# kerry-he/fsae-mpc

Hardware: AMD Instinct MI355X
Metric: QP solves/sec (batched LTV-MPC, N=40 nx=5 nu=2 fp64) (higher is better)
Workload: dtype f64

## Files before the change

### fsae-mpc_amd/csrc/qp_solver.hip

```cpp
#include <hip/hip_runtime.h>
#include <math.h>
#include <stdint.h>
#include <stdlib.h>
#include <stdio.h>
#include "qp_solver.h"

typedef double v4d __attribute__((ext_vector_type(4)));
typedef double v2d __attribute__((ext_vector_type(2)));

#define DEVINL __device__ __forceinline__
#ifndef QP_SOLVE_REFINE_STEPS
#define QP_SOLVE_REFINE_STEPS 1
#endif
#ifndef QP_FULL_BARRIERS
#define WAVE_SYNC() do { __builtin_amdgcn_fence(__ATOMIC_SEQ_CST, "wavefront"); __builtin_amdgcn_wave_barrier(); } while (0)
#else
#define WAVE_SYNC() __syncthreads()
#endif

namespace {

DEVINL double rl(double v, int src) {
  int lo = __builtin_amdgcn_readlane(__double2loint(v), src);
  int hi = __builtin_amdgcn_readlane(__double2hiint(v), src);
// ... 403 lines not shown
}

template <int T> DEVINL void hx_from_acc(const Ctx& k, const v4d* acc, const double* XV, double* HX) {
  double xr[T][4], xc[T], sc[T], sr[T][4];
#pragma unroll
  for (int I = 0; I < T; ++I) {
    xc[I] = XV[16 * I + k.c]; sc[I] = 0.0;
#pragma unroll
    for (int p = 0; p < 4; ++p) { xr[I][p] = XV[16 * I + k.q + 4 * p]; sr[I][p] = 0.0; }
  }
#pragma unroll
  for (int I = 0; I < T; ++I)
#pragma unroll
    for (int J = I; J < T; ++J) {
      const v4d& h = acc[Tri<T>::idx(I, J)];
#pragma unroll
      for (int p = 0; p < 4; ++p) {
        sc[J] = fma(h[p], xr[I][p], sc[J]);
        if (J > I) sr[I][p] = fma(h[p], xc[J], sr[I][p]);
      }
    }
  WAVE_SYNC();
#pragma unroll
  for (int J = 0; J < T; ++J) { const double v = q_sum(sc[J]); if (k.q == 0) HX[16 * J + k.c] = v; }
  WAVE_SYNC();
#pragma unroll
  for (int I = 0; I < T - 1; ++I)
#pragma unroll
    for (int p = 0; p < 4; ++p) { const double v = grp16_sum(sr[I][p]); if (k.c == 0) HX[16 * I + k.q + 4 * p] += v; }
}

template <int C> struct IC { static constexpr int value = C; };

#ifdef QP_DRAIN_STREAM
template <int T> struct StreamCfg {
  static constexpr int R = 3 * T;
};
template <int T> struct Stream {
  static constexpr int R = StreamCfg<T>::R;
  const char* gnext;
  int half;
  DEVINL void issue(const Ctx& k, int slot) {
    __builtin_amdgcn_global_load_lds((const __attribute__((address_space(1))) void*)(gnext + k.lane * 16),
                                     (__attribute__((address_space(3))) void*)(k.ring + slot * 128), 16, 0, 0);
    gnext += 1024;
  }
  DEVINL void start(const Ctx& k, int c0) {
    gnext = reinterpret_cast<const char*>(k.Aw); half = 0;
#pragma unroll
    for (int t = 0; t < T; ++t) if (t < c0) issue(k, t);
  }
  template <int C> DEVINL void next_pair(const Ctx& k, v2d* b, int cn) {
    asm volatile("s_waitcnt vmcnt(0)" ::: "memory");
    const int other = (half ^ 1) * T;
#pragma unroll
    for (int t = 0; t < T; ++t) if (t < cn) issue(k, other + t);
    asm volatile("" ::: "memory");
#pragma unroll
    for (int t = 0; t < C; ++t) b[t] = *reinterpret_cast<const v2d*>(k.ring + (half * T + t) * 128 + k.lane * 2);
    half ^= 1;
  }
  DEVINL void drain() { asm volatile("s_waitcnt vmcnt(0)" ::: "memory"); }
};
#else
template <int T> struct StreamCfg {
  static constexpr int D = 2 * T;
  static constexpr int R = D + T;
};
template <int T> struct Stream {
  static constexpr int D = StreamCfg<T>::D, R = StreamCfg<T>::R;
  const char* gnext; int slot_i, slot_e;
  DEVINL void issue(const Ctx& k) {
    __builtin_amdgcn_global_load_lds((const __attribute__((address_space(1))) void*)(gnext + k.lane * 16),
                                     (__attribute__((address_space(3))) void*)(k.ring + slot_i * 128), 16, 0, 0);
    gnext += 1024;
    slot_i = slot_i + 1 == R ? 0 : slot_i + 1;
  }
  DEVINL void start(const Ctx& k, int) {
    gnext = reinterpret_cast<const char*>(k.Aw); slot_i = 0; slot_e = 0;
#pragma unroll
    for (int j = 0; j < D; ++j) issue(k);
  }
  template <int C> DEVINL void next_pair(const Ctx& k, v2d* b, int) {
#pragma unroll
    for (int t = 0; t < C; ++t) issue(k);
    asm volatile("s_waitcnt vmcnt(%0)" :: "n"(D) : "memory");
#pragma unroll
    for (int t = 0; t < C; ++t) {
      int sl = slot_e + t; if (sl >= R) sl -= R;
      b[t] = *reinterpret_cast<const v2d*>(k.ring + sl * 128 + k.lane * 2);
    }
    slot_e += C; if (slot_e >= R) slot_e -= R;
  }
  DEVINL void drain() { asm volatile("s_waitcnt vmcnt(0)" ::: "memory"); }
};
#endif

template <int NA> struct CoefStage {
  double reg[NA > 0 ? NA : 1];
  DEVINL void load(const Ctx& k, const double* const* arr, int js) {
    const int jc = js < k.J ? js : k.J - 1;
#pragma unroll
    for (int a = 0; a < NA; ++a) reg[a] = arr[a][jc * 64 + k.lane];
  }
  DEVINL void commit(const Ctx& k) {
#pragma unroll
    for (int a = 0; a < NA; ++a) k.cof[a * 64 + k.lane] = reg[a];
  }
  DEVINL void read_pair(const Ctx& k, int s, v2d* out) const {
#pragma unroll
    for (int a = 0; a < NA; ++a) out[a] = *reinterpret_cast<const v2d*>(k.cof + a * 64 + k.q * 16 + (s & 15));
  }
};

template <int T, int NB> DEVINL void pass_syrk(const Ctx& k, v4d* acc, double* P1, double* P2, double* P3, double* MB) {
  constexpr int NBB = NB > 0 ? NB : 1;
  constexpr int NA = 4 + NB;
  const int JS = k.J * 64;
  const double* arr[NA];
  arr[0] = rowp(k, R_D); arr[1] = rowp(k, R_W1); arr[2] = rowp(k, R_W2); arr[3] = rowp(k, R_W3);
#pragma unroll
  for (int e = 0; e < NB; ++e) arr[4 + e] = k.Ab + (size_t)e * JS;
  double p1[T], p2[T], p3[T];
  double pb[NBB][T], sbb[NBB][NBB], pwb[3][NBB];
#pragma unroll
  for (int t = 0; t < T; ++t) { p1[t] = 0; p2[t] = 0; p3[t] = 0; }
#pragma unroll
  for (int e = 0; e < NBB; ++e) {
#pragma unroll
    for (int t = 0; t < T; ++t) pb[e][t] = 0;
#pragma unroll
    for (int f = 0; f < NBB; ++f) sbb[e][f] = 0;
    pwb[0][e] = pwb[1][e] = pwb[2][e] = 0;
  }
  Stream<T> st;
  CoefStage<NA> cs;
  int tr = 0;
  if (k.ntr > 0) { st.start(k, k.tcs[0]); cs.load(k, arr, 0); }
  auto phase = [&](auto Cc) __attribute__((always_inline)) {
    constexpr int C = decltype(Cc)::value;
    const int tr_end = k.tend[C];
    for (; tr < tr_end; ++tr) {
      if ((tr & 3) == 0) { cs.commit(k); cs.load(k, arr, (tr >> 2) + 1); }
#pragma unroll
      for (int u = 0; u < 2; ++u) {
        v2d b[C], cf[NA];
        st.template next_pair<C>(k, b, u == 0 ? C : (tr + 1 < tr_end ? C : (tr + 1 < k.ntr ? k.tcs[tr + 1] : 0)));
        cs.read_pair(k, 4 * tr + 2 * u, cf);
        asm volatile("" ::: "memory");
#pragma unroll
        for (int h = 0; h < 2; ++h) {
          double a[C], ab[NBB];
          const double dd = cf[0][h], w1 = cf[1][h], w2 = cf[2][h], w3 = cf[3][h];
#pragma unroll
          for (int e = 0; e < NB; ++e) ab[e] = cf[4 + e][h];
#pragma unroll
          for (int t = 0; t < C; ++t) a[t] = dd * b[t][h];
#pragma unroll
          for (int I = 0; I < C; ++I)
#pragma unroll
            for (int Jt = I; Jt < C; ++Jt)
              acc[Tri<T>::idx(I, Jt)] = __builtin_amdgcn_mfma_f64_16x16x4f64(a[I], b[Jt][h], acc[Tri<T>::idx(I, Jt)], 0, 0, 0);
#pragma unroll
          for (int t = 0; t < C; ++t) {
            p1[t] = fma(w1, b[t][h], p1[t]); p2[t] = fma(w2, b[t][h], p2[t]); p3[t] = fma(w3, b[t][h], p3[t]);
          }
#pragma unroll
          for (int e = 0; e < NB; ++e) {
            const double dab = dd * ab[e];
#pragma unroll
            for (int t = 0; t < C; ++t) pb[e][t] = fma(dab, b[t][h], pb[e][t]);
#pragma unroll
            for (int f = e; f < NB; ++f) sbb[e][f] = fma(dab, ab[f], sbb[e][f]);
            pwb[0][e] = fma(w1, ab[e], pwb[0][e]); pwb[1][e] = fma(w2, ab[e], pwb[1][e]); pwb[2][e] = fma(w3, ab[e], pwb[2][e]);
          }
        }
      }
    }
  };
  if constexpr (T >= 1) phase(IC<1>{});
  if constexpr (T >= 2) phase(IC<2>{});
  if constexpr (T >= 3) phase(IC<3>{});
  if constexpr (T >= 4) phase(IC<4>{});
  if constexpr (T >= 5) phase(IC<5>{});
  if constexpr (T >= 6) phase(IC<6>{});
  if constexpr (T >= 7) phase(IC<7>{});
  if constexpr (T >= 8) phase(IC<8>{});
  if (k.ntr > 0) st.drain();
#pragma unroll
  for (int t = 0; t < T; ++t) {
    double v1 = q_sum(p1[t]), v2 = q_sum(p2[t]), v3 = q_sum(p3[t]);
    if (k.q == 0) { P1[16 * t + k.c] = v1; P2[16 * t + k.c] = v2; P3[16 * t + k.c] = v3; }
  }
#pragma unroll
  for (int e = 0; e < NB; ++e) {
#pragma unroll
    for (int t = 0; t < T; ++t) { const double vb = q_sum(pb[e][t]); if (k.q == 0) MB[e * k.np + 16 * t + k.c] = vb; }
    const double v1 = q_sum(pwb[0][e]), v2 = q_sum(pwb[1][e]), v3 = q_sum(pwb[2][e]);
    if (k.lane == 0) { P1[k.nc + e] = v1; P2[k.nc + e] = v2; P3[k.nc + e] = v3; }
#pragma unroll
    for (int f = 0; f < NB; ++f) {
      const double sv = q_sum(f >= e ? sbb[e][f] : sbb[f][e]);
      if (k.lane == 0) MB[e * k.np + k.nc + f] = sv;
    }
  }
}

template <int T, int NB, int NVEC, int FUSE> DEVINL void pass_Av(const Ctx& k, const double* const* vin, double* const* rout, double* Pcor, double* Pcor2 = nullptr, const double* const* cfarr = nullptr) {
  constexpr int NBB = NB > 0 ? NB : 1;
  constexpr int NC = FUSE == 1 ? 6 : (FUSE >= 2 ? 3 : 0);
  constexpr int NA = NC + NB;
  const int JS = k.J * 64;
  const double* arr[NA > 0 ? NA : 1];
  if (FUSE == 1) { arr[0] = rowp(k, R_RPL); arr[1] = rowp(k, R_CB1); arr[2] = rowp(k, R_CC1); arr[3] = rowp(k, R_RPU); arr[4] = rowp(k, R_CB2); arr[5] = rowp(k, R_CC2); }
  if (FUSE >= 2) { arr[0] = cfarr ? cfarr[0] : rowp(k, R_CB1); arr[1] = cfarr ? cfarr[1] : rowp(k, R_RPL); arr[2] = cfarr ? cfarr[2] : rowp(k, R_CC1); }
#pragma unroll
  for (int f = 0; f < NB; ++f) arr[NC + f] = k.Ab + (size_t)f * JS;
  double v[NVEC][T], vb[NVEC][NBB], pc[T], pcb[NBB], pd[FUSE >= 2 ? T : 1], pdb[NBB];
#pragma unroll
  for (int e = 0; e < NVEC; ++e) {
#pragma unroll
    for (int t = 0; t < T; ++t) v[e][t] = vin[e][16 * t + k.c];
#pragma unroll
    for (int f = 0; f < NB; ++f) vb[e][f] = vin[e][k.nc + f];
  }
#pragma unroll
  for (int t = 0; t < T; ++t) pc[t] = 0.0;
#pragma unroll
  for (int f = 0; f < NBB; ++f) { pcb[f] = 0.0; pdb[f] = 0.0; }
#pragma unroll
  for (int t = 0; t < (FUSE >= 2 ? T : 1); ++t) pd[t] = 0.0;
  double keep[NVEC + 1];
#pragma unroll
  for (int e = 0; e < NVEC + 1; ++e) keep[e] = 0.0;
  Stream<T> st;
  CoefStage<NA> cs;
  int tr = 0;
  if (k.ntr > 0) { st.start(k, k.tcs[0]); if (NA > 0) cs.load(k, arr, 0); }
  auto phase = [&](auto Cc) __attribute__((always_inline)) {
    constexpr int C = decltype(Cc)::value;
    const int tr_end = k.tend[C];
    for (; tr < tr_end; ++tr) {
      if (NA > 0 && (tr & 3) == 0) { cs.commit(k); cs.load(k, arr, (tr >> 2) + 1); }
#pragma unroll
      for (int u = 0; u < 2; ++u) {
        v2d b[C], cf[NA > 0 ? NA : 1];
        st.template next_pair<C>(k, b, u == 0 ? C : (tr + 1 < tr_end ? C : (tr + 1 < k.ntr ? k.tcs[tr + 1] : 0)));
        if (NA > 0) cs.read_pair(k, 4 * tr + 2 * u, cf);
        asm volatile("" ::: "memory");
#pragma unroll
        for (int h = 0; h < 2; ++h) {
          const int s = 4 * tr + 2 * u + h;
          const int cc = s & 15;
#pragma unroll
          for (int e = 0; e < NVEC; ++e) {
            double dsum = 0.0;
#pragma unroll
            for (int t = 0; t < C; ++t) dsum = fma(b[t][h], v[e][t], dsum);
            dsum = grp16_sum(dsum);
#pragma unroll
            for (int f = 0; f < NB; ++f) dsum = fma(cf[NC + f][h], vb[e][f], dsum);
            if (k.c == cc) keep[e] = dsum;
            if (FUSE >= 2 && e == 0) {
              const double pen = cf[0][h] * (dsum - cf[1][h]);
              const double ynew = cf[2][h] - pen;
              if (k.c == cc) keep[NVEC] = ynew;
#pragma unroll
              for (int t = 0; t < C; ++t) { pc[t] = fma(ynew, b[t][h], pc[t]); pd[t] = fma(pen, b[t][h], pd[t]); }
#pragma unroll
              for (int f = 0; f < NB; ++f) { pcb[f] = fma(ynew, cf[NC + f][h], pcb[f]); pdb[f] = fma(pen, cf[NC + f][h], pdb[f]); }
            }
            if (FUSE == 1 && e == 0) {
              const double dl_ = dsum + cf[0][h], du_ = cf[3][h] - dsum;
              const double w = dl_ * fma(cf[2][h], dl_, cf[1][h]) - du_ * fma(cf[5][h], du_, cf[4][h]);
#pragma unroll
              for (int t = 0; t < C; ++t) pc[t] = fma(w, b[t][h], pc[t]);
#pragma unroll
              for (int f = 0; f < NB; ++f) pcb[f] = fma(w, cf[NC + f][h], pcb[f]);
            }
          }
          if (cc == 15 || s + 1 == 4 * k.ntr) {
            const int js = s >> 4;
#pragma unroll
            for (int e = 0; e < NVEC; ++e) { rout[e][js * 64 + k.lane] = keep[e]; keep[e] = 0.0; }
            if (FUSE >= 2) { rout[NVEC][js * 64 + k.lane] = keep[NVEC]; keep[NVEC] = 0.0; }
          }
        }
      }
    }
  };
  if constexpr (T >= 1) phase(IC<1>{});
  if constexpr (T >= 2) phase(IC<2>{});
  if constexpr (T >= 3) phase(IC<3>{});
  if constexpr (T >= 4) phase(IC<4>{});
  if constexpr (T >= 5) phase(IC<5>{});
  if constexpr (T >= 6) phase(IC<6>{});
  if constexpr (T >= 7) phase(IC<7>{});
  if constexpr (T >= 8) phase(IC<8>{});
  if (k.ntr > 0) st.drain();
  if (FUSE) {
#pragma unroll
    for (int t = 0; t < T; ++t) {
      double pv = q_sum(pc[t]);
      if (k.q == 0) Pcor[16 * t + k.c] = pv;
    }
#pragma unroll
    for (int f = 0; f < NB; ++f) { const double pv = q_sum(pcb[f]); if (k.lane == 0) Pcor[k.nc + f] = pv; }
  }
  if (FUSE >= 2) {
#pragma unroll
    for (int t = 0; t < T; ++t) {
      double pv = q_sum(pd[t]);
      if (k.q == 0) Pcor2[16 * t + k.c] = pv;
    }
#pragma unroll
    for (int f = 0; f < NB; ++f) { const double pv = q_sum(pdb[f]); if (k.lane == 0) Pcor2[k.nc + f] = pv; }
  }
}

template <int T, int NB> DEVINL void pass_Atw(const Ctx& k, const double* W, double* Pout) {
  constexpr int NBB = NB > 0 ? NB : 1;
  const int JS = k.J * 64;
  double p[T], pbv[NBB];
#pragma unroll
  for (int t = 0; t < T; ++t) p[t] = 0.0;
#pragma unroll
  for (int f = 0; f < NBB; ++f) pbv[f] = 0.0;
  for (int s = 0; s < 4 * k.ntr; ++s) {
    const int ri = (s >> 4) * 64 + k.q * 16 + (s & 15);
    const double w = W[ri];
    const int tr = s >> 2, tc = k.tcs[tr];
    const double* src = k.Aw + ((size_t)k.aoff[tr] + ((s >> 1) & 1) * tc) * 128 + k.lane * 2 + (s & 1);
// ... 308 lines not shown
#define aZL rowp(k, R_ZL)
#define aZU rowp(k, R_ZU)
#define aV rowp(k, R_V)
#define aD rowp(k, R_D)
#define aW1 rowp(k, R_W1)
#define aW2 rowp(k, R_W2)
#define aW3 rowp(k, R_W3)
#define aVA rowp(k, R_VA)
#define aVC rowp(k, R_VC)
#define aRPL rowp(k, R_RPL)
#define aRPU rowp(k, R_RPU)

  auto hx_border = [&](const double* XV) __attribute__((always_inline)) {
    if (NB > 0) {
      WAVE_SYNC();
      double xb[NBB], sb[NBB];
#pragma unroll
      for (int e = 0; e < NB; ++e) { xb[e] = XV[nc + e]; sb[e] = 0.0; }
      for (int h = 0; h < 2; ++h) {
        const int i = lane + 64 * h;
        if (i < n) {
          double add = 0.0;
#pragma unroll
          for (int e = 0; e < NB; ++e) { const double hbi = k.Hb[(size_t)e * k.np + i]; add = fma(hbi, xb[e], add); sb[e] = fma(hbi, XV[i], sb[e]); }
          if (i < nc) HX[i] += add;
        }
      }
#pragma unroll
      for (int e = 0; e < NB; ++e) { const double tot = wave_sum(sb[e]); if (lane == 0) HX[nc + e] = tot; }
    }
  };
  auto hx_full = [&](const double* XV) __attribute__((always_inline)) { hx_tiles<T>(k, XV, HX); hx_border(XV); };

  for (int i = lane; i < k.np; i += 64) { G[i] = gw[i]; EV[i] = Es[i]; R1[i] = 0; R2[i] = 0; DX[i] = 0; }
  int cnt_local = 0, infeas = 0;
  for (int js = 0; js < JT; ++js) {
    const int ix = js * 64 + lane;
    const bool valid = row_valid(k, js);
    double l = aL[ix], u = aU[ix];
    if (valid) {
      if (l > -INFINITY && u < INFINITY) {
        if (l > u) infeas = 1;
        if (!(u > l)) {
          const double eps = 1e-9 * fmax(1.0, fabs(l));
          l -= eps; u += eps; aL[ix] = l; aU[ix] = u;
        }
      }
      cnt_local += (l > -INFINITY) + (u < INFINITY);
    }
    if (js >= J) {
      const int i = (js - J) * 64 + lane;
      if (i < k.np) {
        double xi = 0.0;
        if (P.x_init) { const int ui = i < k.n ? qp_user_index(d, i) : -1; if (ui >= 0) { const double xs = P.x_init[(size_t)b * d.nu + ui] / EV[i]; if (fabs(xs) < INFINITY) xi = xs; } }
        if (valid) { if (l > -INFINITY && xi < l) xi = l; if (u < INFINITY && xi > u) xi = u; }
        X[i] = xi;
      }
    }
  }
  const double cnt = fmax(1.0, wave_sum((double)cnt_local));
  infeas = wave_max((double)infeas) > 0;
  WAVE_SYNC();

  STAMP_DECL
  int flag = 1, it = 0, flag_polished = 0;
  double fval_s = 0.0, merit_s = INFINITY;
  if (infeas) { flag = -2; }
  if (ws[d.off_bad] != 0.0) flag = -1;

  {
    const double* vin[1] = {X}; double* rout[1] = {aV};
    pass_Av<T, NB, 1, 0>(k, vin, rout, nullptr);
    for (int jb = 0; jb < k.JB; ++jb) { const int i = jb * 64 + lane; aV[(J + jb) * 64 + lane] = i < n ? X[i] : 0.0; }
  }
  const double T0 = 10.0, Z0 = 100.0;
  for (int js = 0; js < JT; ++js) {
    const int ix = js * 64 + lane;
    const bool valid = row_valid(k, js);
    const double l = aL[ix], u = aU[ix], v = aV[ix];
    const bool hl = valid && l > -INFINITY, hu = valid && u < INFINITY;
    aTL[ix] = hl ? fmax(v - l, T0) : 1.0;
    aTU[ix] = hu ? fmax(u - v, T0) : 1.0;
    aZL[ix] = hl ? Z0 : 0.0;
    aZU[ix] = hu ? Z0 : 0.0;
    aW3[ix] = (js < J) ? ((hl ? Z0 : 0.0) - (hu ? Z0 : 0.0)) : 0.0;
  }
  WAVE_SYNC();
  {
    hx_full(X);
    pass_Atw<T, NB>(k, aW3, P3);
    WAVE_SYNC();
    for (int jb = 0; jb < k.JB; ++jb) {
      const int i = jb * 64 + lane, ix = (J + jb) * 64 + lane;
      if (i < n) {
        const double r = HX[i] + G[i] - P3[i];
        if (aL[ix] > -INFINITY) aZL[ix] = fmax(r, 0.0) + Z0;
        if (aU[ix] < INFINITY) aZU[ix] = fmax(-r, 0.0) + Z0;
      }
    }
    WAVE_SYNC();
  }

  double saved_merit = INFINITY, best_res = INFINITY;
  int have_saved = 0, stall = 0;
  double* XS = ws + d.off_save;
// ... 214 lines not shown
      border_solve(V);
      vec_rows_load<T>(k, V, yv);
    }
    WAVE_SYNC();
    vec_backward<T, false>(k, acc, YL, yv, V);
#endif
  };

  STAMP(0);
  for (it = 0; flag == 1; ++it) {
    if (it == 0) {
      double s_gap = 0, m_rp = 0;
      for (int js = 0; js < JT; ++js) {
        const int ix = js * 64 + lane;
        row1_body(ix, row_valid(k, js), aL[ix], aU[ix], aV[ix], aTL[ix], aTU[ix], aZL[ix], aZU[ix], s_gap, m_rp);
      }
      gap = wave_sum(s_gap);
      rp_rel = wave_max(m_rp);
      WAVE_SYNC();
    }
    const double mu = gap / cnt;

    STAMP(1);
#ifdef QP_HX_SEPARATE
    hx_full(X);
    STAMP(2);
    acc_init<T>(k, acc);
#else
    acc_init<T>(k, acc);
    hx_from_acc<T>(k, acc, X, HX);
    hx_border(X);
    STAMP(2);
#endif
    pass_syrk<T, NB>(k, acc, P1, P2, P3, MB);
    WAVE_SYNC();
    STAMP(3);
    double fl = 0, m_rd = 0;
    for (int h = 0; h < 2; ++h) {
      const int i = lane + 64 * h;
      if (i < n) {
        const int ix = (J + (i >> 6)) * 64 + (i & 63);
        const double gz = P3[i] + aW3[ix];
        fl += 0.5 * X[i] * HX[i] + G[i] * X[i];
        const double sc = fmax(1.0, fmax(fabs(G[i]), fmax(fabs(HX[i]), fabs(gz))));
        m_rd = fmax(m_rd, fabs(HX[i] + G[i] - gz) / sc);
      }
    }
    const double fval = wave_sum(fl);
    const double rd_rel = wave_max(m_rd);
    const double gap_rel = gap / fmax(1.0, fabs(fval));
    const double merit = (fabs(fval) < INFINITY && fabs(gap_rel) < INFINITY) ? fmax(rd_rel, fmax(rp_rel, gap_rel)) : INFINITY;
    fval_s = fval; merit_s = merit;
    const bool res_ok = merit <= P.tol;
#ifdef QP_DEBUG_DUMP
    if (P.dump && P.dump_stage == 5 && b == P.dump_iter && lane == 0 && it < 120) {
      double* o_ = P.dump + 16 * it;
      o_[0] = merit; o_[1] = rd_rel; o_[2] = rp_rel; o_[3] = gap_rel; o_[4] = mu; o_[5] = fval; o_[6] = (double)have_saved; o_[7] = saved_merit;
    }
#endif
    if (!(merit < INFINITY)) { flag = have_saved ? 2 : -1; break; }
    if (merit <= P.tol_loose && merit < saved_merit) {
      for (int i = lane; i < k.np; i += 64) XS[i] = X[i];
      for (int js = 0; js < JT; ++js) LAMS[js * 64 + lane] = aW3[js * 64 + lane];
      have_saved = 1; saved_merit = merit;
    } else if (merit > P.tol_loose && rp_rel <= P.tol_loose && gap_rel <= P.tol_loose) {
      double dgap = 0, m_rd2 = 0, lamfix[2] = {0.0, 0.0};
      for (int h = 0; h < 2; ++h) {
// ... 25 lines not shown
    for (int h = 0; h < 2; ++h) {
      const int i = lane + 64 * h;
      if (i < k.np) {
        const int ix = (J + (i >> 6)) * 64 + (i & 63);
        R1[i] = i < n ? -(HX[i] + G[i]) + P1[i] + aW1[ix] : 0.0;
        R2[i] = i < n ? P2[i] + aW2[ix] : 0.0;
      }
    }
    STAMP(4);
    if (factor_solve2(it)) {
      flag = (res_ok || have_saved) ? 2 : -1;
      if (flag == -1 && P.polish && rp_rel <= QP_BREAKDOWN_TRY_TOL && gap_rel <= QP_BREAKDOWN_TRY_TOL) flag = 4;
      break;
    }
    STAMP(6);
#ifdef QP_DEBUG_DUMP
    if (P.dump && b == 0 && P.dump_stage == 2 && it == P.dump_iter) {
      for (int i = lane; i < n; i += 64) { P.dump[i] = R1[i]; P.dump[n + i] = R2[i]; }
    }
#endif
    if (res_ok) {
      double dm = 0, xm = 1.0;
      for (int h = 0; h < 2; ++h) {
        const int i = lane + 64 * h;
        if (i < n) { dm = fmax(dm, fabs(R1[i] * EV[i])); xm = fmax(xm, fabs(X[i] * EV[i])); }
      }
      dm = wave_max(dm); xm = wave_max(xm);
      if (dm <= P.tol_x * xm) { flag = 0; break; }
    }
    if (it >= P.max_iter) { flag = have_saved ? 2 : 1; break; }

    {
      const double* vin[2] = {R1, R2}; double* rout[2] = {aVA, aVC};
      pass_Av<T, NB, 2, 1>(k, vin, rout, P1);
      for (int jb = 0; jb < k.JB; ++jb) {
        const int i = jb * 64 + lane;
        aVA[(J + jb) * 64 + lane] = i < n ? R1[i] : 0.0;
        aVC[(J + jb) * 64 + lane] = i < n ? R2[i] : 0.0;
      }
    }
    STAMP(7);
    double a_aff = 1.0, s1 = 0.0, s2 = 0.0;
    auto row2_body = [&](const Slot& r, int js) {
      const bool hl = r.valid && r.l > -INFINITY, hu = r.valid && r.u < INFINITY;
      double w = 0.0;
      if (hl) {
        const double dt = r.va + r.rpl, dz = -r.zl - (r.zl / r.tl) * dt;
        if (dt < 0) a_aff = fmin(a_aff, -r.tl / dt);
        if (dz < 0) a_aff = fmin(a_aff, -r.zl / dz);
        s1 += r.tl * dz + r.zl * dt; s2 += dt * dz;
        w -= dt * dz / r.tl;
      }
      if (hu) {
        const double dt = -r.va + r.rpu, dz = -r.zu - (r.zu / r.tu) * dt;
        if (dt < 0) a_aff = fmin(a_aff, -r.tu / dt);
        if (dz < 0) a_aff = fmin(a_aff, -r.zu / dz);
        s1 += r.tu * dz + r.zu * dt; s2 += dt * dz;
        w += dt * dz / r.tu;
      }
      if (js >= J && js < JT) aW1[r.ix] = w;
    };
    for (int js = 0; js < JT; js += 2) {
      const Slot r0 = load_slot(js), r1 = load_slot(js + 1);
      row2_body(r0, js); row2_body(r1, js + 1);
    }
    a_aff = wave_min(a_aff);
    s1 = wave_sum(s1); s2 = wave_sum(s2);
    const double mu_aff = fmax(0.0, gap + a_aff * (s1 + a_aff * s2)) / cnt;
    double sigma = mu > 0 ? (mu_aff / mu) * (mu_aff / mu) * (mu_aff / mu) : 0.0;
    if (sigma > 1.0) sigma = 1.0;
    {
      const double mu_floor = 1e-5 * P.tol * fmax(1.0, fabs(fval)) / cnt;
      if (mu > 0 && sigma < mu_floor / mu) sigma = fmin(1.0, mu_floor / mu);
    }
    const double smu = sigma * mu;
    const double cw = a_aff >= 0.05 ? 1.0 : 0.0;
    WAVE_SYNC();
    STAMP(8);
    if (cw != 0.0) {
    STAMP(9);
    for (int h = 0; h < 2; ++h) {
      const int i = lane + 64 * h;
      if (i < k.np) { const int ix = (J + (i >> 6)) * 64 + (i & 63); DX[i] = i < n ? P1[i] + aW1[ix] : 0.0; }
    }
    WAVE_SYNC();
    solve1(DX);
    WAVE_SYNC();
    STAMP(10);
    {
      const double* vin[1] = {DX}; double* rout[1] = {aW2};
      pass_Av<T, NB, 1, 0>(k, vin, rout, nullptr);
      for (int jb = 0; jb < k.JB; ++jb) { const int i = jb * 64 + lane; aW2[(J + jb) * 64 + lane] = i < n ? DX[i] : 0.0; }
    }
    STAMP(11);
    } else {
      for (int i = lane; i < k.np; i += 64) DX[i] = 0.0;
      for (int js = 0; js < JT; ++js) aW2[js * 64 + lane] = 0.0;
      WAVE_SYNC();
    }
    for (int h = 0; h < 2; ++h) {
      const int i = lane + 64 * h;
      if (i < n) DX[i] = R1[i] + smu * R2[i] + DX[i];
    }
    double amax = 1e300, bp = 0, bdp = 0, bd = 0, bdd = 0, q1 = 0.0, q2 = 0.0;
    auto row3a_body = [&](const Slot& r, int js) {
      const bool hl = r.valid && r.l > -INFINITY, hu = r.valid && r.u < INFINITY;
      const double dv = r.va + smu * r.vc + r.w2;
      if (js < JT) aVC[r.ix] = dv;
      if (hl) {
        const double dta = r.va + r.rpl, dza = -r.zl - (r.zl / r.tl) * dta;
        const double cl = smu - cw * dta * dza;
        const double dt = dv + r.rpl, dz = -r.zl + cl / r.tl - (r.zl / r.tl) * dt;
        if (dt < 0 && -r.tl / dt < amax) { amax = -r.tl / dt; bp = r.tl; bdp = dt; bd = r.zl; bdd = dz; }
        if (dz < 0 && -r.zl / dz < amax) { amax = -r.zl / dz; bp = r.zl; bdp = dz; bd = r.tl; bdd = dt; }
        q1 += r.tl * dz + r.zl * dt; q2 += dt * dz;
      }
      if (hu) {
        const double dta = -r.va + r.rpu, dza = -r.zu - (r.zu / r.tu) * dta;
        const double cu = smu - cw * dta * dza;
        const double dt = -dv + r.rpu, dz = -r.zu + cu / r.tu - (r.zu / r.tu) * dt;
        if (dt < 0 && -r.tu / dt < amax) { amax = -r.tu / dt; bp = r.tu; bdp = dt; bd = r.zu; bdd = dz; }
        if (dz < 0 && -r.zu / dz < amax) { amax = -r.zu / dz; bp = r.zu; bdp = dz; bd = r.tu; bdd = dt; }
        q1 += r.tu * dz + r.zu * dt; q2 += dt * dz;
      }
// ... 71 lines not shown
    xn = wave_max(xn); zn = wave_max(zn);
    WAVE_SYNC();
    STAMP(12);
    if (xn > 1e13) { flag = rp_prev > 1e-6 ? -2 : (fval < -1e13 ? -3 : -1); break; }
    if (zn > 1e15 && rp_prev > 1e-6) { flag = -2; break; }
    if (stall > (have_saved ? 5 : 25)) { flag = have_saved ? 2 : (rp_prev > 1e-6 ? -2 : (P.polish ? 5 : 1)); break; }
  }

  const bool v_current = flag == 0 || flag == 4;
  if (flag == 2) {
    for (int i = lane; i < k.np; i += 64) X[i] = XS[i];
    for (int js = 0; js < JT; ++js) aW3[js * 64 + lane] = LAMS[js * 64 + lane];
    flag = 0; merit_s = saved_merit;
    WAVE_SYNC();
  } else {
    for (int js = 0; js < JT; ++js) {
      const int ix = js * 64 + lane;
      const bool valid = row_valid(k, js);
      const bool hl = valid && aL[ix] > -INFINITY, hu = valid && aU[ix] < INFINITY;
      aW3[ix] = (hl ? aZL[ix] : 0.0) - (hu ? aZU[ix] : 0.0);
    }
    WAVE_SYNC();
  }
#ifdef QP_DEBUG_DUMP
  if (P.dump && P.dump_stage == 5 && b == P.dump_iter && lane == 0) { double* o_ = P.dump + 16 * 120; o_[4] = (double)flag; for (int i_ = 5; i_ < 48; ++i_) o_[i_] = 0.0; }
#endif
  if ((flag == 0 || flag == 4 || flag == 5) && P.polish) {
    const double rho = 1e6, pin = 1e16, rinv = 1.0 / rho;
    double* PA = rowp(k, R_CB1); double* PB = rowp(k, R_RPL); double* PY = rowp(k, R_CC1); double* PS = rowp(k, R_CB2);
    double* PC = rowp(k, R_RPU); double* PP = rowp(k, R_CC2); double* PZ0 = aW2;
    double* ATR = R1; double* ATP = P3;
    if (!v_current) {
      const double* vin[1] = {X}; double* rout[1] = {aV};
      pass_Av<T, NB, 1, 0>(k, vin, rout, nullptr);
      for (int jb = 0; jb < k.JB; ++jb) { const int i = jb * 64 + lane; aV[(J + jb) * 64 + lane] = i < n ? X[i] : 0.0; }
    }
    for (int js = 0; js < JT; ++js) {
      const int ix = js * 64 + lane;
      const bool valid = row_valid(k, js);
      const double l = aL[ix], u = aU[ix], v = aV[ix], lam = aW3[ix];
      const bool lo = valid && l > -INFINITY && lam > 0 && lam > fabs(v - l);
      const bool up = valid && u < INFINITY && lam < 0 && -lam > fabs(u - v);
      PS[ix] = lo ? 1.0 : (up ? -1.0 : 0.0); PY[ix] = ((lo || up) && js < J) ? lam : 0.0;
    }
    for (int i = lane; i < k.np; i += 64) XS[i] = X[i];
    WAVE_SYNC();
    for (int attempt = 0; attempt < QP_REFINE_ATTEMPTS && flag_polished <= 0; ++attempt) {
    for (int js = 0; js < JT; ++js) {
      const int ix = js * 64 + lane;
      const double sd = PS[ix];
      PA[ix] = sd != 0.0 ? rho : 0.0; PB[ix] = sd > 0 ? aL[ix] : (sd < 0 ? aU[ix] : 0.0);
      aD[ix] = js < J ? PA[ix] : (sd != 0.0 ? pin : 0.0); aW1[ix] = 0.0; aW2[ix] = 0.0; PC[ix] = 0.0; PP[ix] = 0.0;
    }
    WAVE_SYNC();
    acc_init<T>(k, acc);
    pass_syrk<T, NB>(k, acc, P1, P2, P3, MB);
    WAVE_SYNC();
    for (int i = lane; i < k.np; i += 64) { R1[i] = 0.0; R2[i] = 0.0; }
    WAVE_SYNC();
    bool pok = factor_solve2(-1) == 0, retry = false;
    if (!pok) { flag_polished = -5; break; }
    for (int h = 0; h < 2; ++h) {
      const int i = lane + 64 * h;
      if (i < k.np) { const int ix = (J + (i >> 6)) * 64 + (i & 63); R2[i] = (i < n && PS[ix] != 0.0) ? PB[ix] : XS[i]; }
    }
    WAVE_SYNC();
    const double* cf_eval[3] = {PA, PB, PY};
    const double* cf_cg[3] = {PA, PZ0, PZ0};
    auto eval_zy = [&]() __attribute__((always_inline)) {
      const double* vin[1] = {R2}; double* rout[2] = {aVA, aVC};
      pass_Av<T, NB, 1, 3>(k, vin, rout, P1, P2, cf_eval);
      hx_full(R2);
      WAVE_SYNC();
    };
    if (pok) {
      eval_zy();
      for (int h = 0; h < 2; ++h) {
        const int i = lane + 64 * h;
        if (i < k.np) { const int ix = (J + (i >> 6)) * 64 + (i & 63); DX[i] = (i < n && PS[ix] == 0.0) ? -(HX[i] + G[i] - P1[i]) : 0.0; }
      }
      WAVE_SYNC();
      solve1(DX);
      WAVE_SYNC();
      for (int h = 0; h < 2; ++h) {
        const int i = lane + 64 * h;
        if (i < n) { const int ix = (J + (i >> 6)) * 64 + (i & 63); if (PS[ix] == 0.0) R2[i] += DX[i]; }
      }
      WAVE_SYNC();
      eval_zy();
      double rs_l = 0.0;
      for (int js = 0; js < J; ++js) {
        const int ix = js * 64 + lane;
        const double cc_ = PA[ix] != 0.0 ? aVA[ix] - PB[ix] : 0.0;
        PC[ix] = cc_; PP[ix] = -cc_; rs_l = fma(cc_, cc_, rs_l);
      }
      double rs = wave_sum(rs_l);
      for (int h = 0; h < 2; ++h) { const int i = lane + 64 * h; if (i < k.np) { ATR[i] = -P2[i] * rinv; ATP[i] = ATR[i]; } }
      WAVE_SYNC();
      for (int cgit = 0; cgit < 12 && pok; ++cgit) {
        double m_eq = 0.0, m_cy = 0.0;
        for (int js = 0; js < J; ++js) {
          const int ix = js * 64 + lane;
          m_eq = fmax(m_eq, fabs(PC[ix]) / fmax(1.0, fabs(PB[ix])));
          m_cy = fmax(m_cy, fabs(PC[ix] * PY[ix]));
        }
        m_eq = wave_max(m_eq); m_cy = wave_max(m_cy);
        if (m_eq <= 1e-11 && m_cy <= 1e-11 * fmax(1.0, fabs(fval_s))) break;
        if (cgit == 11) { pok = false; flag_polished = -6; break; }
        for (int h = 0; h < 2; ++h) {
          const int i = lane + 64 * h;
          if (i < k.np) { const int ix = (J + (i >> 6)) * 64 + (i & 63); DX[i] = (i < n && PS[ix] == 0.0) ? ATP[i] : 0.0; }
        }
        WAVE_SYNC();
        solve1(DX);
        WAVE_SYNC();
        {
          const double* vin[1] = {DX}; double* rout[2] = {aVA, aVC};
          pass_Av<T, NB, 1, 3>(k, vin, rout, P1, P2, cf_cg);
        }
        WAVE_SYNC();
        double pq_l = 0.0;
        for (int js = 0; js < J; ++js) { const int ix = js * 64 + lane; if (PA[ix] != 0.0) pq_l = fma(PP[ix], aVA[ix], pq_l); }
        const double pq = wave_sum(pq_l);
        if (!(pq > 0.0) || !(rs > 0.0)) {
          pok = false; flag_polished = -7;
          if (attempt < QP_REFINE_ATTEMPTS - 1) {
            double my = 0.0; int myix = -1;
            for (int js = 0; js < J; ++js) { const int ix = js * 64 + lane; if (PA[ix] != 0.0 && fabs(PP[ix]) > my) { my = fabs(PP[ix]); myix = ix; } }
            const double mx = wave_max(my);
            if (mx > 0.0 && my == mx && myix >= 0) { PS[myix] = 0.0; PY[myix] = 0.0; }
            for (int i = lane; i < k.np; i += 64) XS[i] = R2[i];
            WAVE_SYNC();
            retry = true;
          }
          break;
        }
        const double alpha_ = rs / pq;
        double rsn_l = 0.0;
        for (int js = 0; js < J; ++js) {
          const int ix = js * 64 + lane;
          if (PA[ix] != 0.0) {
            PY[ix] = fma(alpha_, PP[ix], PY[ix]);
            const double cc_ = fma(alpha_, aVA[ix], PC[ix]);
            PC[ix] = cc_; rsn_l = fma(cc_, cc_, rsn_l);
          }
        }
        const double rsn = wave_sum(rsn_l);
        const double beta_ = rsn / rs;
        for (int js = 0; js < J; ++js) { const int ix = js * 64 + lane; if (PA[ix] != 0.0) PP[ix] = fma(beta_, PP[ix], -PC[ix]); }
        for (int h = 0; h < 2; ++h) {
          const int i = lane + 64 * h;
// ... 100 lines not shown
        fval_s = f2; merit_s = fmax(m_rd, fmax(m_rp, m_cp / fmax(1.0, fabs(f2))));
        flag = 0;
      }
      WAVE_SYNC();
    } else if (!retry) break;
    }
  }
  if (flag == 4) flag = -1;
  if (flag == 5) flag = 1;
  double* xo = P.x + (size_t)b * d.nu;
  for (int i = lane; i < n; i += 64) { const int ui = qp_user_index(d, i); if (ui >= 0) xo[ui] = X[i] * EV[i]; }
  if (P.lambda) {
    double* lo = P.lambda + (size_t)b * (d.nu + k.m);
    for (int jb = 0; jb < k.JB; ++jb) {
      const int i = jb * 64 + lane;
      const int ui = i < n ? qp_user_index(d, i) : -1;
      if (ui >= 0) lo[ui] = aW3[(J + jb) * 64 + lane] / EV[i];
    }
    for (int js = 0; js < J; ++js) {
      const int r = k.perm[js * 64 + lane];
      if (r >= 0) lo[d.nu + r] = aW3[js * 64 + lane] * Fs[js * 64 + lane];
    }
  }
  if (!(v_current || flag_polished > 0)) {
    WAVE_SYNC();
    hx_full(X);
    WAVE_SYNC();
    double fl = 0;
    for (int h = 0; h < 2; ++h) { const int i = lane + 64 * h; if (i < n) fl += 0.5 * X[i] * HX[i] + G[i] * X[i]; }
    fval_s = wave_sum(fl);
  }
  STAMP(13);
  STAMP_OUT;
#ifdef QP_DEBUG_DUMP
  if (P.dump && P.dump_stage == 5 && b == P.dump_iter && lane == 0) { double* o_ = P.dump + 16 * 120; o_[0] = (double)flag; o_[1] = (double)it; o_[2] = (double)flag_polished; o_[3] = merit_s; }
#endif
  if (lane == 0) {
    P.fval[b] = fval_s;
    P.exitflag[b] = flag;
    P.iter[b] = it;
    if (P.polished) P.polished[b] = flag_polished;
    if (P.kkt) P.kkt[b] = merit_s;
  }
}

#undef aL
#undef aU
#undef aTL
#undef aTU
#undef aZL
#undef aZU
#undef aV
#undef aD
#undef aW1
#undef aW2
#undef aW3
#undef aVA
#undef aVC
#undef aRPL
#undef aRPU
#undef X
#undef G
#undef HX
#undef R1
#undef R2
#undef P1
// ... 12 lines not shown
  for (int p = 0; p < 4; ++p) Cm[((lane >> 4) + 4 * p) * 16 + (lane & 15)] = c[p];
}
#endif

}

#if QP_MAIN_TU

#ifdef QP_PROBE
template <int T, int NB> __global__ __launch_bounds__(64) void syrk_probe_kernel(QpParams P, int reps) {
  const int b = blockIdx.x;
  Ctx k;
  const QpDims& d = P.d;
  k.n = d.n; k.m = d.m; k.T = T; k.Kq = d.Kq; k.J = d.J; k.JB = d.JB; k.JT = d.J + d.JB; k.np = d.np; k.ld = 0;
  k.lane = threadIdx.x; k.c = k.lane & 15; k.q = k.lane >> 4; k.nc = d.nc; k.nb = d.nb;
  double* ws = P.ws + (size_t)b * d.ws_per_qp;
  k.Aw = ws + d.off_Aw; k.Hw = ws + d.off_Hw; k.Ab = ws + d.off_Ab; k.Hb = ws + d.off_Hb;
  k.rows = ws + d.off_rows; k.rowlen = d.rowlen; k.ntr = d.ntr;
  k.perm = reinterpret_cast<const int*>(ws + d.off_meta); k.tcs = k.perm + (size_t)(d.J > 0 ? d.J : 1) * 64;
  k.aoff = k.tcs + d.ntr; k.tend = k.aoff + d.ntr + 1;
  extern __shared__ double lds[];
  k.Ms = nullptr; k.vec = lds;
  double* MB = lds + (size_t)V_NARR * d.np;
  k.ring = MB + (size_t)(NB > 0 ? NB : 1) * d.np + T * 272; k.cof = k.ring + StreamCfg<T>::R * 128;
  for (int js = 0; js < k.JT; ++js) {
    const int ix = js * 64 + k.lane;
    rowp(k, R_D)[ix] = 1.0; rowp(k, R_W1)[ix] = 0.5; rowp(k, R_W2)[ix] = 0.25; rowp(k, R_W3)[ix] = 2.0;
  }
  __syncthreads();
  v4d acc[Tri<T>::NT];
  acc_init<T>(k, acc);
  const unsigned long long t0 = __builtin_amdgcn_s_memtime();
  for (int r = 0; r < reps; ++r) {
    pass_syrk<T, NB>(k, acc, vecp(k, V_P1), vecp(k, V_P2), vecp(k, V_P3), MB);
    __syncthreads();
  }
  const unsigned long long t1 = __builtin_amdgcn_s_memtime();
  double cs = 0;
#pragma unroll
  for (int i = 0; i < Tri<T>::NT; ++i) cs += acc[i][0] + acc[i][1] + acc[i][2] + acc[i][3];
  cs = wave_sum(cs);
  if (k.lane == 0) { P.dump[b] = (double)(t1 - t0) / reps; P.dump[gridDim.x + b] = cs; }
}
#endif

#ifdef QP_PROBE
template <int T> __global__ __launch_bounds__(64) void factor_probe_kernel(QpParams P, int reps) {
  const int b = blockIdx.x;
  Ctx k;
  const QpDims& d = P.d;
  k.n = d.n; k.m = d.m; k.T = T; k.Kq = d.Kq; k.J = d.J; k.JB = d.JB; k.JT = d.J + d.JB; k.np = d.np; k.ld = 0;
  k.lane = threadIdx.x; k.c = k.lane & 15; k.q = k.lane >> 4; k.nc = d.nc; k.nb = d.nb;
  double* ws = P.ws + (size_t)b * d.ws_per_qp;
  k.Aw = ws + d.off_Aw; k.Hw = ws + d.off_Hw; k.Ab = ws + d.off_Ab; k.Hb = ws + d.off_Hb;
  k.rows = ws + d.off_rows; k.rowlen = d.rowlen; k.ntr = d.ntr;
  extern __shared__ double lds[];
  k.Ms = nullptr; k.vec = lds;
  double* MB = lds + (size_t)V_NARR * d.np;
  double* YL = MB + (size_t)1 * d.np;
  k.ring = YL + T * 272; k.cof = k.ring + StreamCfg<T>::R * 128;
  double* SCR = k.ring;
  v4d acc[Tri<T>::NT], rh[T];
  unsigned long long tt[4] = {0, 0, 0, 0};
  double cs = 0;
  for (int r = 0; r < reps; ++r) {
    acc_init<T>(k, acc);
#pragma unroll
// ... 254 lines not shown
```

Measured before the change: 375,100.

## Hoist global-to-LDS stream state across passes with optional carry-over prefetch

Moves the Stream object out of each pass into the solver so its state persists, caches the trip-end table in wave-uniform scalars via readfirstlane, and adds an opt-in QP_STREAM_CARRY mode. In that mode the ring keeps prefetching wrapped-around records of the constraint matrix across pass boundaries instead of draining and refilling per pass. By default (carry undefined) behaviour is nearly unchanged apart from uniform-scalarized tend values and a guard on the initial issue. Carry mode risks stale ring slots if other code touches the ring between passes.

```diff
diff --git a/fsae-mpc_amd/csrc/qp_solver.hip b/fsae-mpc_amd/csrc/qp_solver.hip
--- a/fsae-mpc_amd/csrc/qp_solver.hip
+++ b/fsae-mpc_amd/csrc/qp_solver.hip
@@ -459,6 +459,15 @@
 
 template <int C> struct IC { static constexpr int value = C; };
 
+#if defined(QP_STREAM_CARRY) && (defined(QP_DRAIN_STREAM) || defined(QP_MFMA_SOLVES))
+#error "QP_STREAM_CARRY: the full-drain ring restarts per pass by construction, and the MFMA solves use the ring as scratch between passes"
+#endif
+DEVINL int uni(int v) { return __builtin_amdgcn_readfirstlane(v); }
+DEVINL const char* uni(const char* p) {
+  const unsigned long long v = reinterpret_cast<unsigned long long>(p);
+  const unsigned lo = __builtin_amdgcn_readfirstlane((unsigned)v), hi = __builtin_amdgcn_readfirstlane((unsigned)(v >> 32));
+  return reinterpret_cast<const char*>(((unsigned long long)hi << 32) | lo);
+}
 #ifdef QP_DRAIN_STREAM
 template <int T> struct StreamCfg {
   static constexpr int R = 3 * T;
@@ -467,13 +476,21 @@
   static constexpr int R = StreamCfg<T>::R;
   const char* gnext;
   int half;
+  int tend[T + 1];
   DEVINL void issue(const Ctx& k, int slot) {
     __builtin_amdgcn_global_load_lds((const __attribute__((address_space(1))) void*)(gnext + k.lane * 16),
                                      (__attribute__((address_space(3))) void*)(k.ring + slot * 128), 16, 0, 0);
     gnext += 1024;
   }
-  DEVINL void start(const Ctx& k, int c0) {
+  DEVINL void open(const Ctx& k) {
+#pragma unroll
+    for (int C = 0; C <= T; ++C) tend[C] = uni(k.tend[C]);
+  }
+  DEVINL void start(const Ctx& k) {
+#pragma unroll
+    for (int C = 0; C <= T; ++C) tend[C] = uni(tend[C]);
     gnext = reinterpret_cast<const char*>(k.Aw); half = 0;
+    const int c0 = k.ntr > 0 ? k.tcs[0] : 0;
 #pragma unroll
     for (int t = 0; t < T; ++t) if (t < c0) issue(k, t);
   }
@@ -487,7 +504,8 @@
     for (int t = 0; t < C; ++t) b[t] = *reinterpret_cast<const v2d*>(k.ring + (half * T + t) * 128 + k.lane * 2);
     half ^= 1;
   }
-  DEVINL void drain() { asm volatile("s_waitcnt vmcnt(0)" ::: "memory"); }
+  DEVINL void finish() { asm volatile("s_waitcnt vmcnt(0)" ::: "memory"); }
+  DEVINL void close() { asm volatile("s_waitcnt vmcnt(0)" ::: "memory"); }
 };
 #else
 template <int T> struct StreamCfg {
@@ -496,21 +514,57 @@
 };
 template <int T> struct Stream {
   static constexpr int D = StreamCfg<T>::D, R = StreamCfg<T>::R;
-  const char* gnext; int slot_i, slot_e;
+  const char* gnext; int slot_i, slot_e, left, nrec;
+  int tend[T + 1];
   DEVINL void issue(const Ctx& k) {
     __builtin_amdgcn_global_load_lds((const __attribute__((address_space(1))) void*)(gnext + k.lane * 16),
                                      (__attribute__((address_space(3))) void*)(k.ring + slot_i * 128), 16, 0, 0);
     gnext += 1024;
     slot_i = slot_i + 1 == R ? 0 : slot_i + 1;
   }
-  DEVINL void start(const Ctx& k, int) {
+  DEVINL void issue_wrap(const Ctx& k) {
+    issue(k);
+    if (--left == 0) { gnext = reinterpret_cast<const char*>(k.Aw); left = nrec; }
+  }
+  DEVINL void open(const Ctx& k) {
+    gnext = reinterpret_cast<const char*>(k.Aw); slot_i = 0; slot_e = 0; left = nrec = 0;
+#pragma unroll
+    for (int C = 0; C <= T; ++C) tend[C] = uni(k.tend[C]);
+#ifdef QP_STREAM_CARRY
+    if (k.ntr > 0) {
+      left = nrec = uni(k.aoff[k.ntr]);
+#pragma unroll
+      for (int j = 0; j < D; ++j) issue_wrap(k);
+    }
+#endif
+  }
+  DEVINL void start(const Ctx& k) {
+#ifndef QP_STREAM_CARRY
     gnext = reinterpret_cast<const char*>(k.Aw); slot_i = 0; slot_e = 0;
-#pragma unroll
-    for (int j = 0; j < D; ++j) issue(k);
+    if (k.ntr > 0) {
+#pragma unroll
+      for (int j = 0; j < D; ++j) issue(k);
+    }
+#else
+    gnext = uni(gnext); slot_i = uni(slot_i); slot_e = uni(slot_e); left = uni(left); nrec = uni(nrec);
+#endif
+#pragma unroll
+    for (int C = 0; C <= T; ++C) tend[C] = uni(tend[C]);
   }
   template <int C> DEVINL void next_pair(const Ctx& k, v2d* b, int) {
+#ifndef QP_STREAM_CARRY
 #pragma unroll
     for (int t = 0; t < C; ++t) issue(k);
+#else
+    if (left > C) {
+#pragma unroll
+      for (int t = 0; t < C; ++t) issue(k);
+      left -= C;
+    } else {
+#pragma unroll
+      for (int t = 0; t < C; ++t) issue_wrap(k);
+    }
+#endif
     asm volatile("s_waitcnt vmcnt(%0)" :: "n"(D) : "memory");
 #pragma unroll
     for (int t = 0; t < C; ++t) {
@@ -519,7 +573,12 @@
     }
     slot_e += C; if (slot_e >= R) slot_e -= R;
   }
-  DEVINL void drain() { asm volatile("s_waitcnt vmcnt(0)" ::: "memory"); }
+  DEVINL void finish() {
+#if !defined(QP_STREAM_CARRY) || defined(QP_STREAM_PASS_DRAIN)
+    asm volatile("s_waitcnt vmcnt(0)" ::: "memory");
+#endif
+  }
+  DEVINL void close() { asm volatile("s_waitcnt vmcnt(0)" ::: "memory"); }
 };
 #endif
 
@@ -540,7 +599,7 @@
   }
 };
 
-template <int T, int NB> DEVINL void pass_syrk(const Ctx& k, v4d* acc, double* P1, double* P2, double* P3, double* MB) {
+template <int T, int NB> DEVINL void pass_syrk(const Ctx& k, Stream<T>& st, v4d* acc, double* P1, double* P2, double* P3, double* MB) {
   constexpr int NBB = NB > 0 ? NB : 1;
   constexpr int NA = 4 + NB;
   const int JS = k.J * 64;
@@ -560,13 +619,13 @@
     for (int f = 0; f < NBB; ++f) sbb[e][f] = 0;
     pwb[0][e] = pwb[1][e] = pwb[2][e] = 0;
   }
-  Stream<T> st;
   CoefStage<NA> cs;
   int tr = 0;
-  if (k.ntr > 0) { st.start(k, k.tcs[0]); cs.load(k, arr, 0); }
+  st.start(k);
+  if (k.ntr > 0) cs.load(k, arr, 0);
   auto phase = [&](auto Cc) __attribute__((always_inline)) {
     constexpr int C = decltype(Cc)::value;
-    const int tr_end = k.tend[C];
+    const int tr_end = st.tend[C];
     for (; tr < tr_end; ++tr) {
       if ((tr & 3) == 0) { cs.commit(k); cs.load(k, arr, (tr >> 2) + 1); }
 #pragma unroll
@@ -613,7 +672,7 @@
   if constexpr (T >= 6) phase(IC<6>{});
   if constexpr (T >= 7) phase(IC<7>{});
   if constexpr (T >= 8) phase(IC<8>{});
-  if (k.ntr > 0) st.drain();
+  if (k.ntr > 0) st.finish();
 #pragma unroll
   for (int t = 0; t < T; ++t) {
     double v1 = q_sum(p1[t]), v2 = q_sum(p2[t]), v3 = q_sum(p3[t]);
@@ -633,7 +692,7 @@
   }
 }
 
-template <int T, int NB, int NVEC, int FUSE> DEVINL void pass_Av(const Ctx& k, const double* const* vin, double* const* rout, double* Pcor, double* Pcor2 = nullptr, const double* const* cfarr = nullptr) {
+template <int T, int NB, int NVEC, int FUSE> DEVINL void pass_Av(const Ctx& k, Stream<T>& st, const double* const* vin, double* const* rout, double* Pcor, double* Pcor2 = nullptr, const double* const* cfarr = nullptr) {
   constexpr int NBB = NB > 0 ? NB : 1;
   constexpr int NC = FUSE == 1 ? 6 : (FUSE >= 2 ? 3 : 0);
   constexpr int NA = NC + NB;
@@ -660,13 +719,13 @@
   double keep[NVEC + 1];
 #pragma unroll
   for (int e = 0; e < NVEC + 1; ++e) keep[e] = 0.0;
-  Stream<T> st;
   CoefStage<NA> cs;
   int tr = 0;
-  if (k.ntr > 0) { st.start(k, k.tcs[0]); if (NA > 0) cs.load(k, arr, 0); }
+  st.start(k);
+  if (k.ntr > 0 && NA > 0) cs.load(k, arr, 0);
   auto phase = [&](auto Cc) __attribute__((always_inline)) {
     constexpr int C = decltype(Cc)::value;
-    const int tr_end = k.tend[C];
+    const int tr_end = st.tend[C];
     for (; tr < tr_end; ++tr) {
       if (NA > 0 && (tr & 3) == 0) { cs.commit(k); cs.load(k, arr, (tr >> 2) + 1); }
 #pragma unroll
@@ -724,7 +783,7 @@
   if constexpr (T >= 6) phase(IC<6>{});
   if constexpr (T >= 7) phase(IC<7>{});
   if constexpr (T >= 8) phase(IC<8>{});
-  if (k.ntr > 0) st.drain();
+  if (k.ntr > 0) st.finish();
   if (FUSE) {
 #pragma unroll
     for (int t = 0; t < T; ++t) {
@@ -1099,6 +1158,9 @@
   };
   auto hx_full = [&](const double* XV) __attribute__((always_inline)) { hx_tiles<T>(k, XV, HX); hx_border(XV); };
 
+  Stream<T> st;
+  st.open(k);
+
   for (int i = lane; i < k.np; i += 64) { G[i] = gw[i]; EV[i] = Es[i]; R1[i] = 0; R2[i] = 0; DX[i] = 0; }
   int cnt_local = 0, infeas = 0;
   for (int js = 0; js < JT; ++js) {
@@ -1137,7 +1199,7 @@
 
   {
     const double* vin[1] = {X}; double* rout[1] = {aV};
-    pass_Av<T, NB, 1, 0>(k, vin, rout, nullptr);
+    pass_Av<T, NB, 1, 0>(k, st, vin, rout, nullptr);
     for (int jb = 0; jb < k.JB; ++jb) { const int i = jb * 64 + lane; aV[(J + jb) * 64 + lane] = i < n ? X[i] : 0.0; }
   }
   const double T0 = 10.0, Z0 = 100.0;
@@ -1418,7 +1480,7 @@
     hx_border(X);
     STAMP(2);
 #endif
-    pass_syrk<T, NB>(k, acc, P1, P2, P3, MB);
+    pass_syrk<T, NB>(k, st, acc, P1, P2, P3, MB);
     WAVE_SYNC();
     STAMP(3);
     double fl = 0, m_rd = 0;
@@ -1510,7 +1572,7 @@
 
     {
       const double* vin[2] = {R1, R2}; double* rout[2] = {aVA, aVC};
-      pass_Av<T, NB, 2, 1>(k, vin, rout, P1);
+      pass_Av<T, NB, 2, 1>(k, st, vin, rout, P1);
       for (int jb = 0; jb < k.JB; ++jb) {
         const int i = jb * 64 + lane;
         aVA[(J + jb) * 64 + lane] = i < n ? R1[i] : 0.0;
@@ -1567,7 +1629,7 @@
     STAMP(10);
     {
       const double* vin[1] = {DX}; double* rout[1] = {aW2};
-      pass_Av<T, NB, 1, 0>(k, vin, rout, nullptr);
+      pass_Av<T, NB, 1, 0>(k, st, vin, rout, nullptr);
       for (int jb = 0; jb < k.JB; ++jb) { const int i = jb * 64 + lane; aW2[(J + jb) * 64 + lane] = i < n ? DX[i] : 0.0; }
     }
     STAMP(11);
@@ -1705,7 +1767,7 @@
     double* ATR = R1; double* ATP = P3;
     if (!v_current) {
       const double* vin[1] = {X}; double* rout[1] = {aV};
-      pass_Av<T, NB, 1, 0>(k, vin, rout, nullptr);
+      pass_Av<T, NB, 1, 0>(k, st, vin, rout, nullptr);
       for (int jb = 0; jb < k.JB; ++jb) { const int i = jb * 64 + lane; aV[(J + jb) * 64 + lane] = i < n ? X[i] : 0.0; }
     }
     for (int js = 0; js < JT; ++js) {
@@ -1727,7 +1789,7 @@
     }
     WAVE_SYNC();
     acc_init<T>(k, acc);
-    pass_syrk<T, NB>(k, acc, P1, P2, P3, MB);
+    pass_syrk<T, NB>(k, st, acc, P1, P2, P3, MB);
     WAVE_SYNC();
     for (int i = lane; i < k.np; i += 64) { R1[i] = 0.0; R2[i] = 0.0; }
     WAVE_SYNC();
@@ -1742,7 +1804,7 @@
     const double* cf_cg[3] = {PA, PZ0, PZ0};
     auto eval_zy = [&]() __attribute__((always_inline)) {
       const double* vin[1] = {R2}; double* rout[2] = {aVA, aVC};
-      pass_Av<T, NB, 1, 3>(k, vin, rout, P1, P2, cf_eval);
+      pass_Av<T, NB, 1, 3>(k, st, vin, rout, P1, P2, cf_eval);
       hx_full(R2);
       WAVE_SYNC();
     };
@@ -1789,7 +1851,7 @@
         WAVE_SYNC();
         {
           const double* vin[1] = {DX}; double* rout[2] = {aVA, aVC};
-          pass_Av<T, NB, 1, 3>(k, vin, rout, P1, P2, cf_cg);
+          pass_Av<T, NB, 1, 3>(k, st, vin, rout, P1, P2, cf_cg);
         }
         WAVE_SYNC();
         double pq_l = 0.0;
@@ -1956,6 +2018,7 @@
   }
   STAMP(13);
   STAMP_OUT;
+  st.close();
 #ifdef QP_DEBUG_DUMP
   if (P.dump && P.dump_stage == 5 && b == P.dump_iter && lane == 0) { double* o_ = P.dump + 16 * 120; o_[0] = (double)flag; o_[1] = (double)it; o_[2] = (double)flag_polished; o_[3] = merit_s; }
 #endif
@@ -2034,7 +2097,10 @@
   acc_init<T>(k, acc);
   const unsigned long long t0 = __builtin_amdgcn_s_memtime();
   for (int r = 0; r < reps; ++r) {
-    pass_syrk<T, NB>(k, acc, vecp(k, V_P1), vecp(k, V_P2), vecp(k, V_P3), MB);
+    Stream<T> st;
+    st.open(k);
+    pass_syrk<T, NB>(k, st, acc, vecp(k, V_P1), vecp(k, V_P2), vecp(k, V_P3), MB);
+    st.close();
     __syncthreads();
   }
   const unsigned long long t1 = __builtin_amdgcn_s_memtime();
```

New measurement: 379,700, median of 6. 1.01x the previous value.
